# peakcrosser7/spmv-samples

Measured on AMD Instinct MI355X. Metric: GFLOP/s (2*nnz/t) and achieved HBM GB/s, CSR SpMV fp32, 1/2/4/8 MI355X, higher is better.
Workload: dtype f32

## Files before the change

include/mi355_spmv.h:

```cpp
#ifndef MI355_SPMV_H
#define MI355_SPMV_H

#include <stddef.h>
#include <stdint.h>

#ifdef __cplusplus
extern "C" {
#endif

#define MI355_SPMV_VERSION 310
#define MI355_SPMV_HAS_PATTERN 1
#define MI355_SPMV_HAS_MULTI 1
#define MI355_SPMV_HAS_MULTI_SEMIRING 1
#define MI355_SPMV_HAS_MULTI_HALF 1
#define MI355_SPMV_HAS_HALF_MATRIX 1

enum {
    MI355_SPMV_OK = 0,
    MI355_SPMV_EINVAL = 1,
    MI355_SPMV_ENOTSUP = 2,
    MI355_SPMV_EHIP = 3,
    MI355_SPMV_ENOMEM = 4,
    MI355_SPMV_ENODEV = 5
};
// ... 82 lines not shown
    int64_t grid_blocks;
    int64_t tile_items;
    int64_t n_tiles;
    int64_t rows_per_chunk;
    int64_t scratch_bytes;
    int32_t n_kernels;
    int32_t window_elems;
    int32_t window_segments;
    char main_kernel[64];
    int32_t balanced_chunks;
    int32_t rows_cap;
    int64_t n_chunks;
    char knobs[160];
    int64_t packed_index_bytes;
    int64_t packed_index_escapes;
} mi355_spmv_plan_info;
int mi355_spmv_plan_get_info(const mi355_spmv_plan* plan, mi355_spmv_plan_info* info);

typedef struct mi355_spmv_plan_shape {
    int32_t struct_bytes;
    int32_t kind, off_type, val_type;
    int32_t n_rows, n_cols;
    int64_t nnz;
    int32_t lanes_per_row, elems_per_lane, block_threads;
    int32_t balanced_chunks, rows_cap, giant_rows_enabled;
    int64_t rows_per_chunk, n_chunks, bal_k, bal_q, giant_len;
    int32_t window_elems, window_bytes, window_from_band, window_segments, probe_ok, long_steps;
    int64_t band_lo, band_hi, seg_lo[4], seg_hi[4];
    int32_t window_sweep;
    int32_t small_plain;
// ... 162 lines not shown
```

spmv-samples_amd/capi.py:

```python
import ctypes as C
import os

import torch

_HERE = os.path.dirname(os.path.abspath(__file__))
LIB_PATH = os.environ.get("MI355_SPMV_LIB") or os.path.join(_HERE, "lib", "libmi355spmv.so")

KINDS = {"vector": 0, "merge": 1, "light": 2, "auto": 100}
KIND_NAMES = {0: "vector", 1: "merge", 2: "light"}
LABELS = {"hip_vector": "vector", "hip_merge": "merge", "hip_light": "light", "hip_auto": "auto"}
OFF_TYPES = {torch.int32: (0, "i32"), torch.int64: (1, "i64")}
VAL_TYPES = {torch.float32: (0, "f32"), torch.float64: (1, "f64"), torch.int32: (2, "i32")}
VAL_PATTERN = 3
MAT_TYPES = {torch.float16: (4, "f16"), torch.bfloat16: (5, "bf16")}
PLAN_REUSE_STRUCTURE = 1
PLAN_NO_INDEX_COPY = 2
SEMIRINGS = {"plus_times": 0, "min_plus": 1, "max_times": 2, "max_plus": 3, "or_and": 4}

EXPORTS = (
    ["mi355_spmv_%s_%s_%s" % (k, o, v) for k in KINDS for o in ("i32", "i64") for v in ("f32", "f64")]
    + ["mi355_spmv_merge_genl_%s_%s" % (o, v) for o in ("i32", "i64") for v in ("f32", "f64", "i32")]
    + ["mi355_spmv_plan_set_semiring", "mi355_spmv_plan_set_alpha_beta"]
    + ["mi355_spmv_plan_create", "mi355_spmv_plan_execute", "mi355_spmv_plan_destroy",
       "mi355_spmv_plan_get_info", "mi355_spmv_stream_synchronize", "mi355_spmv_plan_merge_coords", "mi355_spmv_version",
# ... 14 lines not shown
    + ["mi355_spmv_multi_%s_%s" % (o, v) for o in ("i32", "i64") for v in ("f32", "f64")]
    + ["mi355_spmv_multi_" + n for n in ("create_typed", "set_semiring", "get_types")]
    + ["mi355_spmv_multi_%s_%s_%s" % (g, o, v) for g in ("genl", "pattern") for o in ("i32", "i64") for v in ("f32", "f64", "i32")]
    + ["mi355_spmv_multi_create_half"]
    + ["mi355_spmv_multi_half_%s_%s" % (o, v) for o in ("i32", "i64") for v in ("f16", "bf16")]
)


class PlanInfo(C.Structure):
    _fields_ = [("kind", C.c_int32), ("off_type", C.c_int32), ("val_type", C.c_int32),
                ("lanes_per_row", C.c_int32), ("elems_per_lane", C.c_int32), ("block_threads", C.c_int32),
                ("grid_blocks", C.c_int64), ("tile_items", C.c_int64), ("n_tiles", C.c_int64),
                ("rows_per_chunk", C.c_int64), ("scratch_bytes", C.c_int64), ("n_kernels", C.c_int32),
                ("window_elems", C.c_int32), ("window_segments", C.c_int32), ("main_kernel", C.c_char * 64),
                ("balanced_chunks", C.c_int32), ("rows_cap", C.c_int32), ("n_chunks", C.c_int64),
                ("knobs", C.c_char * 160), ("packed_index_bytes", C.c_int64), ("packed_index_escapes", C.c_int64)]

    def as_dict(self):
        d = {n: getattr(self, n) for n, _ in self._fields_}
        d["main_kernel"] = d["main_kernel"].decode()
        d["knobs"] = d["knobs"].decode()
        return d


class PlanShape(C.Structure):
    _fields_ = [("struct_bytes", C.c_int32), ("kind", C.c_int32), ("off_type", C.c_int32), ("val_type", C.c_int32),
                ("n_rows", C.c_int32), ("n_cols", C.c_int32), ("nnz", C.c_int64),
                ("lanes_per_row", C.c_int32), ("elems_per_lane", C.c_int32), ("block_threads", C.c_int32),
                ("balanced_chunks", C.c_int32), ("rows_cap", C.c_int32), ("giant_rows_enabled", C.c_int32),
                ("rows_per_chunk", C.c_int64), ("n_chunks", C.c_int64), ("bal_k", C.c_int64), ("bal_q", C.c_int64),
                ("giant_len", C.c_int64),
# ... 803 lines not shown
```

spmv-samples_amd/csrc/capi.hip:

```cpp

#include <algorithm>
#include <cstdarg>
#include <mutex>
#include <new>
#include <type_traits>

#include "common.hpp"

struct mi355_spmv_plan {
    mi355::Plan p;
    int acquired_on = -1;
    int asked_kind = -1;
};

namespace mi355 {

static thread_local char g_err[512] = "";

void set_error(const char* fmt, ...) {
    va_list ap;
    va_start(ap, fmt);
    vsnprintf(g_err, sizeof(g_err), fmt, ap);
    va_end(ap);
}
// ... 495 lines not shown
    if (!h || !info) { set_error("plan_get_info: null argument"); return MI355_SPMV_EINVAL; }
    const Plan& p = h->p;
    memset(info, 0, sizeof(*info));
    info->kind = p.kind; info->off_type = p.off_type; info->val_type = p.val_type;
    info->lanes_per_row = p.lanes_per_row;
    info->elems_per_lane = p.elems_per_lane;
    info->block_threads = (p.kind == MI355_KIND_MERGE && p.merge_rows && p.mat_type != MI355_VAL_PATTERN)
                              ? p.mr_block : (p.block_threads > 0 ? p.block_threads : kBlock);
    info->grid_blocks = p.grid_blocks;
    info->tile_items = p.tile_items;
    info->n_tiles = p.n_tiles;
    info->rows_per_chunk = p.rows_per_chunk;
    info->scratch_bytes = (int64_t)(p.scratch_bytes + p.packed_bytes);
    info->packed_index_bytes = (int64_t)p.packed_bytes;
    info->packed_index_escapes = p.packed_escapes;
    info->n_kernels = p.n_kernels;
    const bool windowed = p.window_elems > 0 && !(is_half_matrix(p.mat_type) && !half_matrix_chunked(p));
    info->window_elems = windowed ? p.window_elems : 0;
    info->window_segments = windowed ? (p.n_seg >= 2 ? p.n_seg : 1) : 0;
    snprintf(info->main_kernel, sizeof(info->main_kernel), "%s", p.main_kernel);
    info->balanced_chunks = p.balanced ? 1 : 0;
    info->rows_cap = p.rows_cap;
    info->n_chunks = p.n_chunks;
    snprintf(info->knobs, sizeof(info->knobs), "%s", p.knob.text);
    return MI355_SPMV_OK;
}

int mi355_spmv_plan_get_mat_type(const mi355_spmv_plan* h, int* mat_type) {
    if (!h || !mat_type) { set_error("plan_get_mat_type: null argument"); return MI355_SPMV_EINVAL; }
    *mat_type = h->p.mat_type;
// ... 105 lines not shown
```

spmv-samples_amd/csrc/common.hpp:

```cpp
#pragma once

#include <hip/hip_runtime.h>

#include <cstdint>
#include <cstdio>
#include <cstring>
#include <mutex>

#include "../../include/mi355_spmv.h"

namespace mi355 {

constexpr int kWave = 64;
constexpr int kBlock = 256;
constexpr int kMaxGiantRows = 1024;
constexpr int64_t kGiantRow = 65536;
constexpr int64_t kGiantSlice = 32768;
inline int64_t giant_slice_for(int64_t giant_len) {
    int64_t s = (giant_len / 2) & ~int64_t(1023);
    if (s < 2048) s = 2048;
    return s < kGiantSlice ? s : kGiantSlice;
}
constexpr int kWideBlock = 512;
constexpr int kHugeBlock = 1024;
// ... 116 lines not shown
    int n_giant = 0;
    int64_t giant_len = 0;
    int64_t n_giant_slices = 0;
    int32_t* giant_row = nullptr;
    int64_t* giant_slice_first = nullptr;
    void* giant_partial = nullptr;
    void* scratch = nullptr;
    size_t scratch_bytes = 0;
    size_t scratch_capacity = 0;
    int32_t* tile_row = nullptr;
    int64_t* tile_nnz = nullptr;
    int32_t* carry_row = nullptr;
    void* carry_val = nullptr;
    unsigned long long* counters = nullptr;
    uint16_t* packed_index = nullptr;
    size_t packed_bytes = 0;
    int64_t packed_escapes = 0;
    bool light_dequeue_once = false;
    int n_kernels = 0;
    bool small_plain = false;
    char main_kernel[64] = "";
};
static_assert(sizeof(Plan) <= 2048, "Plan (1 096 bytes) holds what executes and reports read; plan-time buffers are locals of plan_create");

constexpr int kProbePerRow = 32;
struct ProbeSamples {
    int n = 0;
    bool sorted = false;
    int64_t off[kBlock * kProbePerRow];
};
struct GiantRowList {
    int32_t row[kMaxGiantRows];
    int64_t slice_first[kMaxGiantRows + 1];
};
struct BlockSpec {
    const mi355_spmv_plan_shape* whole;
    int64_t row_begin, chunk_begin, n_chunks, nnz_begin_whole;
    int phase;
// ... 57 lines not shown
```

spmv-samples_amd/csrc/csr_vector.hip:

```cpp

#include <cstdlib>

#include "common.hpp"
#include "row_dot.hpp"
#include "row_launch.hpp"
#include "xwindow.hpp"

namespace mi355 {

template <int BLOCK, int T, int R, int NSEG, bool ADAPT, typename val_t, bool PACKED = false>
__global__ __launch_bounds__(BLOCK, (BLOCK >= kWideBlock || R == 2 ? 4 : 3)) void csr_vector_window_kernel(
    int32_t n_rows, int32_t n_cols, int64_t nnz, const ApView Ap, const int32_t* __restrict__ Aj,
    const val_t* __restrict__ Ax, const val_t* __restrict__ x, val_t* __restrict__ y, ChunkMap cmap,
    int32_t window_cap, BandHint hint, SegmentPlan segs, const uint16_t* __restrict__ Aj16, val_t alpha, val_t beta) {
    static_assert(!PACKED || (NSEG == 1 && !ADAPT), "the packed index exists for one band-placed window and equal-row chunks");
    extern __shared__ __attribute__((aligned(16))) unsigned char s_dyn[];
    __shared__ int s_red[2];
    ChunkScratch<val_t> scr(s_dyn, window_cap, cmap.rows_cap);
    scr.alpha = alpha;
    scr.beta = beta;
    scr.long_steps = cmap.long_steps;
    scr.giant_len = cmap.giant_len;
    const unsigned chunk = cmap.table ? blockIdx.x : xcd_contiguous_id(blockIdx.x, gridDim.x);
    int64_t rb, re;
    cmap.range(chunk, n_rows, rb, re);
    if (rb >= re) return;
    bool fits;
    const int64_t base = stage_chunk_bounds<val_t>(scr, rb, re, Ap, cmap.rel_limit, fits);
    if (!fits) {
// ... 7 lines not shown
    const int32_t nnz_c = int32_t(left < kRel32Limit + 32768 ? left : kRel32Limit + 32768);
    if constexpr (NSEG > 1) {
        auto stage = [&] { return stage_x_segments<val_t>(rb, re, n_cols, x, scr.s_x, window_cap, segs); };
        chunk_rows_any<BLOCK, T, R, true, ADAPT, val_t>(rb, re, nnz_c, Aj_c, Ax_c, x, y, stage, scr);
    } else {
        auto first_last = [&](int64_t r, int& first, int& last) {
            const int32_t s = scr.s_b[r - rb], e = scr.s_b[r - rb + 1];
            if (e <= s) return false;
            first = Aj_c[s];
            last = Aj_c[e - 1];
            return true;
        };
        auto stage = [&] {
            return stage_x_window<val_t>(rb, re, n_cols, first_last, x, scr.s_x, window_cap, s_red, hint);
        };
        if constexpr (PACKED)
            chunk_rows_any<BLOCK, T, R, true, false, val_t, decltype(stage)&, false, true>(rb, re, nnz_c, Aj_c, Ax_c, x, y, stage,
                                                                                          scr, Aj16 + base);
        else
            chunk_rows_any<BLOCK, T, R, NSEG == 1, ADAPT, val_t>(rb, re, nnz_c, Aj_c, Ax_c, x, y, stage, scr);
    }
}

template <int T, int R, typename val_t>
__global__ __launch_bounds__(kHugeBlock, 4) void csr_vector_sweep_kernel(
    int32_t n_rows, int32_t n_cols, int64_t nnz, const ApView Ap, const int32_t* __restrict__ Aj,
    const val_t* __restrict__ Ax, const val_t* __restrict__ x, val_t* __restrict__ y, ChunkMap cmap,
    int32_t window_cap, BandHint hint, val_t alpha, val_t beta) {
    extern __shared__ __attribute__((aligned(16))) unsigned char s_dyn[];
    ChunkScratch<val_t> scr(s_dyn, window_cap, cmap.rows_cap);
    scr.alpha = alpha;
    scr.beta = beta;
// ... 25 lines not shown
    off_t start = 0, end = 0;
    if (live) {
        start = Ap[row];
        end = Ap[row + 1];
    }
    val_t sum = row_partial<T, off_t, val_t>(start, end, lane, Aj, Ax, x);
    sum = vector_reduce<T, val_t>(sum);
    if (live && lane == 0) y[row] = (beta != val_t(0)) ? alpha * sum + beta * y[row] : alpha * sum;
}

struct VectorRows {
    static constexpr const char* name = "csr_vector";
    static constexpr bool kCounters = false;
    static constexpr bool kPlainKnob = true;
    static constexpr bool kPackedIndex = true;
    template <int BLOCK, int T, int R, int NSEG, bool ADAPT, typename val_t, bool PACKED = false>
    static auto window() { return csr_vector_window_kernel<BLOCK, T, R, NSEG, ADAPT, val_t, PACKED>; }
    template <int T, int R, typename val_t>
    static auto sweep() { return csr_vector_sweep_kernel<T, R, val_t>; }
    template <typename off_t, typename val_t>
    static int plain(const Plan& p, const off_t* Ap, const val_t* Ax, const val_t* x, val_t* y, hipStream_t s) {
        return launch_vector_plain<off_t, val_t>(p, Ap, Ax, x, y, s);
    }
};

template <typename off_t, typename val_t>
int launch_vector_plain(const Plan& p, const off_t* Ap, const val_t* Ax, const val_t* x, val_t* y, hipStream_t s) {
    return with_lanes(p, VectorRows::name, [&](auto lanes) -> int {
        constexpr int T = decltype(lanes)::value, rows_per_block = kBlock / T;
        const dim3 grid((unsigned)((int64_t(p.n_rows) + rows_per_block - 1) / rows_per_block)), block(kBlock);
        hipLaunchKernelGGL((csr_vector_kernel<T, off_t, val_t>), grid, block, 0, s, p.n_rows, (off_t)p.nnz, Ap, p.Aj, Ax, x, y,
                           (val_t)p.alpha, (val_t)p.beta);
// ... 20 lines not shown
```

spmv-samples_amd/csrc/csr_vector_h16.hip:

```cpp

#include "common.hpp"
#include "row_dot.hpp"
#include "row_launch.hpp"
#include "xwindow.hpp"

namespace mi355 {
namespace h16 {

template <int BLOCK, int T, int R, int NSEG, bool PACKED, typename mat_t>
__global__ __launch_bounds__(BLOCK, (BLOCK >= kWideBlock || R == 2 ? 4 : 3)) void csr_vector_window_kernel(
    int32_t n_rows, int32_t n_cols, int64_t nnz, const ApView Ap, const int32_t* __restrict__ Aj,
    const mat_t* __restrict__ Ax, const float* __restrict__ x, float* __restrict__ y, ChunkMap cmap,
    int32_t window_cap, BandHint hint, const uint16_t* __restrict__ Aj16, float alpha, float beta) {
    static_assert(NSEG == 0 || NSEG == 1, "one window of x or none");
    static_assert(!PACKED || NSEG == 1, "the packed index exists for one band-placed window");
    extern __shared__ __attribute__((aligned(16))) unsigned char s_dyn[];
    __shared__ int s_red[2];
    ChunkScratch<float> scr(s_dyn, window_cap, cmap.rows_cap);
    scr.alpha = alpha;
    scr.beta = beta;
    scr.long_steps = cmap.long_steps;
    scr.giant_len = cmap.giant_len;
    const unsigned chunk = xcd_contiguous_id(blockIdx.x, gridDim.x);
    int64_t rb, re;
    cmap.range(chunk, n_rows, rb, re);
    if (rb >= re) return;
    bool fits;
    const int64_t base = stage_chunk_bounds<float>(scr, rb, re, Ap, cmap.rel_limit, fits);
    if (!fits) {
// ... 1 lines not shown
        return;
    }
    __syncthreads();
    const int32_t* const Aj_c = Aj + base;
    const mat_t* const Ax_c = Ax + base;
    const int64_t left = nnz - base;
    const int32_t nnz_c = int32_t(left < kRel32Limit + 32768 ? left : kRel32Limit + 32768);
    auto first_last = [&](int64_t r, int& first, int& last) {
        const int32_t s = scr.s_b[r - rb], e = scr.s_b[r - rb + 1];
        if (e <= s) return false;
        first = Aj_c[s];
        last = Aj_c[e - 1];
        return true;
    };
    auto stage = [&] { return stage_x_window<float>(rb, re, n_cols, first_last, x, scr.s_x, window_cap, s_red, hint); };
    chunk_rows_any<BLOCK, T, R, NSEG == 1, false, float, decltype(stage)&, false, PACKED>(rb, re, nnz_c, Aj_c, Ax_c, x, y, stage, scr,
                                                                                          PACKED ? Aj16 + base : nullptr);
}

template <int T, typename off_t, typename mat_t>
__global__ __launch_bounds__(kBlock) void csr_vector_kernel(
    int32_t n_rows, off_t nnz, const off_t* __restrict__ Ap, const int32_t* __restrict__ Aj,
    const mat_t* __restrict__ Ax, const float* __restrict__ x, float* __restrict__ y, float alpha, float beta) {
    constexpr int ROWS_PER_BLOCK = kBlock / T;
    const unsigned blk = xcd_contiguous_id(blockIdx.x, gridDim.x);
    const int lane = threadIdx.x & (T - 1);
    const int64_t row = int64_t(blk) * ROWS_PER_BLOCK + (threadIdx.x / T);
    const bool live = row < n_rows;
    off_t start = 0, end = 0;
    if (live) {
        start = Ap[row];
        end = Ap[row + 1];
// ... 33 lines not shown
        return MI355_SPMV_OK;
    });
}

template <int BLOCK, typename mat_t>
static int launch_window(const RowOperands<float, mat_t>& o) {
    const Plan& p = o.p;
    if constexpr (BLOCK >= kWideBlock) {
        if (p.window_elems <= 0) return launch_window<kBlock, mat_t>(o);
    }
    const BandHint hint{p.band_lo, p.band_hi, p.window_from_band};
    const ChunkMap cmap = chunk_map_of(p);
    auto go = [&](auto kernel) { return launch_chunked<Rows, float>(kernel, BLOCK, o, cmap, hint, (const uint16_t*)p.packed_index); };
    return with_lanes(p, Rows::name, [&](auto lanes) -> int {
        constexpr int T = decltype(lanes)::value, R = rows_in_flight(sizeof(float), T);
        if (p.packed_index && p.window_elems > 0 && p.window_from_band) return go(csr_vector_window_kernel<BLOCK, T, R, 1, true, mat_t>);
        if (p.window_elems > 0) return go(csr_vector_window_kernel<BLOCK, T, R, 1, false, mat_t>);
        if constexpr (BLOCK == kBlock) return go(csr_vector_window_kernel<BLOCK, T, R, 0, false, mat_t>);
        return MI355_SPMV_OK;
    });
}

}

template <typename off_t, typename mat_t>
int launch_vector_half(const Plan& p, const off_t* Ap, const mat_t* Ax, const float* x, float* y, hipStream_t s) {
    static_assert(sizeof(mat_t) == 2, "a 16-bit stored type");
    if (p.n_rows == 0) return MI355_SPMV_OK;
    const bool aligned = ((reinterpret_cast<uintptr_t>(p.Aj) | reinterpret_cast<uintptr_t>(x)) & 15u) == 0 &&
                         (reinterpret_cast<uintptr_t>(Ax) & 7u) == 0;
    if (!half_matrix_chunked(p) || !aligned || p.nnz < 4 || (p.knob.plain != 0 && !p.is_block))
        return h16::launch_plain<off_t, mat_t>(p, Ap, Ax, x, y, s);
    const RowOperands<float, mat_t> o{p, ApView{Ap, sizeof(off_t) == 8 ? 1 : 0}, Ax, x, y, s,
// ... 24 lines not shown
```

spmv-samples_amd/csrc/row_dot.hpp:

```cpp
#pragma once

#include <type_traits>

#include "common.hpp"

namespace mi355 {

typedef int int4v __attribute__((ext_vector_type(4)));
typedef unsigned uint2v __attribute__((ext_vector_type(2)));
constexpr unsigned kPackedEscape = 0xFFFFu;
typedef float float4v __attribute__((ext_vector_type(4)));
typedef double double4v __attribute__((ext_vector_type(4)));

template <typename val_t> struct Vec4;
template <> struct Vec4<float> { using type = float4v; };
template <> struct Vec4<double> { using type = double4v; };
template <> struct Vec4<int32_t> { using type = int4v; };
template <> struct Vec4<PatternOnes> { using type = PatternOnes; };

typedef _Float16 half4v __attribute__((ext_vector_type(4)));
template <> struct Vec4<_Float16> { using type = uint2v; };
template <> struct Vec4<Bf16> { using type = uint2v; };

template <typename val_t, typename mat_t>
// ... 45 lines not shown
```

spmv-samples_amd/csrc/row_launch.hpp:

```cpp

#pragma once

#include <type_traits>

#include "common.hpp"
#include "giant_rows.hpp"
#include "xwindow.hpp"

namespace mi355 {

template <typename F>
static int with_lanes(const Plan& p, const char* kind, F&& f) {
    switch (p.lanes_per_row) {
        case 2: return f(std::integral_constant<int, 2>());
        case 4: return f(std::integral_constant<int, 4>());
        case 8: return f(std::integral_constant<int, 8>());
        case 16: return f(std::integral_constant<int, 16>());
        case 32: return f(std::integral_constant<int, 32>());
        case 64: return f(std::integral_constant<int, 64>());
    }
    set_error("%s: bad lanes_per_row %d", kind, p.lanes_per_row);
    return MI355_SPMV_EINVAL;
}

// ... 45 lines not shown
        constexpr int R = rows_in_flight(sizeof(val_t), 2);
        const int st = p.window_elems > 0 ? go(Kind::template window<kBlock, 2, R, 1, true, val_t>())
                                          : go(Kind::template window<kBlock, 2, R, 0, true, val_t>());
        if (st != MI355_SPMV_OK) return st;
        return launch_giant_rows<off_t, val_t>(p, Ap, o.Ax, o.x, o.y, o.s);
    }
    return with_lanes(p, Kind::name, [&](auto lanes) -> int {
        constexpr int T = decltype(lanes)::value, R = rows_in_flight(sizeof(val_t), T);
        if (p.window_elems > 0 && p.n_seg >= 2) {
            if constexpr (BLOCK == kBlock) return go(Kind::template window<BLOCK, T, R, kMaxSegments, false, val_t>());
            set_error("%s: no 512-thread kernel for a multi-band window", Kind::name);
            return MI355_SPMV_EINVAL;
        }
        if constexpr (Kind::kPackedIndex) {
            if (p.packed_index && p.window_elems > 0 && p.window_from_band)
                return go(Kind::template window<BLOCK, T, R, 1, false, val_t, true>());
        }
        if (p.window_elems > 0) return go(Kind::template window<BLOCK, T, R, 1, false, val_t>());
        if constexpr (BLOCK == kBlock) return go(Kind::template window<BLOCK, T, R, 0, false, val_t>());
        return MI355_SPMV_OK;
    });
}

template <typename Kind, typename val_t>
static int launch_rows_sweep(const RowOperands<val_t>& o) {
    const Plan& p = o.p;
    const BandHint hint{p.band_lo, p.band_hi, true};
    const ChunkMap cmap{nullptr, (int32_t)p.rows_per_chunk, (int32_t)p.rows_cap, p.n_chunks, 0, int64_t(0),
                        p.knob.rel32_limit > 0 ? p.knob.rel32_limit : kRel32Limit, p.light_dequeue_once ? 1 : 0};
    const int64_t vectors = kHugeBlock / p.lanes_per_row;
    const int held = int(p.rows_per_chunk / vectors);
// ... 33 lines not shown
```

spmv-samples_amd/csrc/rows_plan.hip:

```cpp

#include <algorithm>
#include <utility>

#include "common.hpp"
#include "row_dot.hpp"
#include "xwindow.hpp"

namespace mi355 {

static int workgroups_per_cu_by_registers(const Plan& p) {
    if (p.block_threads == kHugeBlock) return 1;
    if (p.block_threads == kWideBlock) return 2;
    if (p.balanced) return p.val_type == MI355_VAL_F64 ? 4 : 3;
    return (p.val_type == MI355_VAL_F64 || p.lanes_per_row >= 16) ? 4 : 3;
}

int long_steps_for(const Plan& p) {
    if (p.knob.long_steps > 0) return p.knob.long_steps;
    return p.balanced ? 4 : kLongSteps;
}

static int pick_lanes_per_row(int64_t nnz, int64_t n_rows, int elems) {
    const int64_t mean = n_rows > 0 ? (nnz + n_rows - 1) / n_rows : 0;
    int t = 2;
// ... 226 lines not shown
    const int tid = threadIdx.x;
    if (tid < s4 - s) out[s + tid] = uint16_t(encode(Aj[s + tid]));
    if (tid < e - e4) out[e4 + tid] = uint16_t(encode(Aj[e4 + tid]));
    for (int64_t k = s4 + int64_t(tid) * 4; k < e4; k += int64_t(kBlock) * 4) {
        const int4v c = stream_load(reinterpret_cast<const int4v*>(Aj + k));
        uint2v v;
        v[0] = encode(c[0]) | (encode(c[1]) << 16);
        v[1] = encode(c[2]) | (encode(c[3]) << 16);
        *reinterpret_cast<uint2v*>(out + k) = v;
    }
#pragma unroll
    for (int o = 32; o >= 1; o >>= 1) escaped += __shfl_xor(escaped, o, kWave);
    if ((tid & (kWave - 1)) == 0 && escaped) atomicAdd(escapes, (unsigned long long)escaped);
}

int build_packed_index(Plan& p) {
    p.packed_index = nullptr;
    p.packed_bytes = 0;
    p.packed_escapes = 0;
    if (p.kind != MI355_KIND_VECTOR || (p.flags & MI355_PLAN_NO_INDEX_COPY) || p.knob.pack == 0) return MI355_SPMV_OK;
    if (p.small_plain || p.sweep || p.balanced || (p.knob.plain != 0 && !p.is_block)) return MI355_SPMV_OK;
    if (p.window_elems <= 0 || p.window_elems > 65535 || p.n_seg >= 2 || !p.window_from_band) return MI355_SPMV_OK;
    if (p.n_rows <= 0 || p.nnz < 4 || p.nnz <= p.nnz_begin || p.n_chunks < 1 || p.n_chunks > int64_t(UINT32_MAX)) return MI355_SPMV_OK;
    if ((reinterpret_cast<uintptr_t>(p.Aj) & 15u) != 0) return MI355_SPMV_OK;
    const size_t bytes = (((size_t(p.nnz_read) + 3) & ~size_t(3)) + 4) * sizeof(uint16_t);
    void* ptr = nullptr;
    if (hipMalloc(&ptr, bytes) != hipSuccess) {
        (void)hipGetLastError();
        return MI355_SPMV_OK;
    }
    const AnalysisBuffer buf;
    unsigned long long* d_escapes = reinterpret_cast<unsigned long long*>(buf.words);
    hipError_t e = d_escapes ? hipSuccess : hipErrorOutOfMemory;
    if (e == hipSuccess) e = hipMemsetAsync(ptr, 0xFF, bytes, nullptr);
    if (e == hipSuccess) e = hipMemsetAsync(d_escapes, 0, sizeof(unsigned long long), nullptr);
    if (e == hipSuccess) {
        const ApView Ap{p.Ap, p.off_type == MI355_OFF_I64 ? 1 : 0};
        const BandHint hint{p.band_lo, p.band_hi, true};
        const dim3 grid((unsigned)p.n_chunks), block(kBlock);
        if (p.val_type == MI355_VAL_F64)
            hipLaunchKernelGGL((pack_index_kernel<double>), grid, block, 0, nullptr, p.n_rows, p.n_cols, Ap, p.Aj,
                               static_cast<uint16_t*>(ptr), chunk_map_of(p), (int32_t)p.window_elems, hint, d_escapes);
        else
            hipLaunchKernelGGL((pack_index_kernel<float>), grid, block, 0, nullptr, p.n_rows, p.n_cols, Ap, p.Aj,
                               static_cast<uint16_t*>(ptr), chunk_map_of(p), (int32_t)p.window_elems, hint, d_escapes);
        e = hipGetLastError();
    }
    unsigned long long escaped = 0;
    if (e == hipSuccess) e = hipMemcpy(&escaped, d_escapes, sizeof(escaped), hipMemcpyDeviceToHost);
    if (e != hipSuccess) {
        (void)hipFree(ptr);
        set_error("build_packed_index: %s", hipGetErrorString(e));
        return MI355_SPMV_EHIP;
    }
    p.packed_index = static_cast<uint16_t*>(ptr);
    p.packed_bytes = bytes;
    p.packed_escapes = int64_t(escaped);
    return MI355_SPMV_OK;
}

static int window_budget(const Plan& p, int block_threads, int64_t rows) {
    if (block_threads == kBlock) return kWindowBytes;
    const size_t val_bytes = p.val_type == MI355_VAL_F64 ? 8 : 4;
    const int64_t avail = 63 * 1024 - int64_t(chunk_lds_bytes(0, int(rows), val_bytes));
    return int(avail < 0 ? 0 : avail);
}

static int rows_in_flight_of(const Plan& p) { return rows_in_flight(p.val_type == MI355_VAL_F64 ? 8 : 4, p.lanes_per_row); }
static bool one_band_window(const Plan& p) { return p.window_elems > 0 && p.n_seg < 2 && p.window_from_band; }

static void shrink_to_whole_rounds(Plan& p, int64_t pass) {
    if (p.knob.rows_per_chunk > 0 || p.n_seg >= 2) return;
// ... 271 lines not shown
```

spmv-samples_amd/csrc/xwindow.hpp:

```cpp
#pragma once

#include <climits>
#include <type_traits>

#include "common.hpp"
#include "row_dot.hpp"

namespace mi355 {

constexpr int kSamples = 32;

template <typename val_t>
struct XWindow {
    const val_t* s_x;
    int32_t lo;
    int32_t len;
    __device__ __forceinline__ bool find(int32_t col, unsigned& idx) const {
        const unsigned rel = unsigned(col - lo);
        const bool in = rel < unsigned(len);
        idx = in ? rel : 0u;
        return in;
    }
};

// ... 319 lines not shown
        for (int g = tid; g < full; g += BLOCK)
            __builtin_nontemporal_store(*reinterpret_cast<const v16*>(scr.s_y + g * PER16),
                                        reinterpret_cast<v16*>(yc + g * PER16));
        for (int i = full * PER16 + tid; i < n_store; i += BLOCK) yc[i] = scr.s_y[i];
    } else if (!scaled) {
        for (int i = tid; i < n_store; i += BLOCK) yc[i] = scr.s_y[i];
    } else {
        for (int i = tid; i < n_store; i += BLOCK) {
            val_t v = alpha * scr.s_y[i];
            if (beta != val_t(0)) v += beta * yc[i];
            yc[i] = v;
        }
    }
}

template <int BLOCK, int T, int R, bool WINDOW, typename val_t, bool PACKED = false, typename StageFn, typename mat_t = val_t>
__device__ __forceinline__ void chunk_rows(int64_t chunk_begin, int64_t chunk_end, int32_t nnz,
                                           const int32_t* __restrict__ Aj,
                                           const mat_t* __restrict__ Ax, const val_t* __restrict__ x,
                                           val_t* __restrict__ y, StageFn&& stage,
                                           const ChunkScratch<val_t>& scr,
                                           const uint16_t* __restrict__ Aj16 = nullptr) {
    static_assert(!PACKED || WINDOW, "a packed index is window-relative");
    using v4 = typename Vec4<val_t>::type;
    using m4 = typename Vec4<mat_t>::type;
    using col4 = typename std::conditional<PACKED, uint2v, int4v>::type;
    using off_t = int32_t;
    constexpr int VECS = BLOCK / T;
    constexpr int WAVES = BLOCK / kWave;
    constexpr int STRIDE = VECS * R;
    const off_t LONG = off_t(T) * 4 * scr.long_steps;
    const int lane = threadIdx.x & (T - 1);
    const int rows = int(chunk_end - chunk_begin);
    const int n_groups = (rows + STRIDE - 1) / STRIDE;
    const off_t nnz_vec = nnz & ~off_t(3);
    const off_t j_max = nnz_vec - 4;

    constexpr int VW = kWave / T;
    const int row_in_wave = (threadIdx.x & (kWave - 1)) / T;
    const int wave_rows0 = (threadIdx.x / kWave) * (VW * R);
#ifdef MI355_ROW_MAP_ADJACENT
    auto row_of = [&](int g, int r) { return g * STRIDE + int(threadIdx.x / T) * R + r; };
#else
    auto row_of = [&](int g, int r) { return g * STRIDE + wave_rows0 + r * VW + row_in_wave; };
#endif
    struct Group {
        col4 c[R];
        m4 a[R];
    };
    auto load_cols = [&](off_t jl) {
        if constexpr (PACKED) return stream_load(reinterpret_cast<const uint2v*>(Aj16 + jl));
        else return stream_load(reinterpret_cast<const int4v*>(Aj + jl));
    };
    struct Bounds { off_t lo[R], hi[R]; };
    auto read_bounds = [&](int g, Bounds& B) {
#pragma unroll
        for (int r = 0; r < R; ++r) {
            const int row = row_of(g, r);
            B.lo[r] = scr.s_b[min(row, rows)];
            B.hi[r] = scr.s_b[min(row + 1, rows)];
        }
    };
    auto step0 = [&](off_t lo) { return (lo & ~off_t(3)) + off_t(lane) * 4; };
    auto issue = [&](int g, Group& G) {
        Bounds B;
        read_bounds(g, B);
#pragma unroll
        for (int r = 0; r < R; ++r) {
            const off_t j0 = step0(B.lo[r]);
            off_t jl = j0 < B.hi[r] ? j0 : (B.lo[r] & ~off_t(3));
            jl = jl < j_max ? jl : j_max;
            G.c[r] = load_cols(jl);
            G.a[r] = stream_load(reinterpret_cast<const m4*>(Ax + jl));
        }
        __builtin_amdgcn_sched_barrier(0);
    };
    constexpr int DEPTH = 2;
    Group G[DEPTH];
#pragma unroll
    for (int d = 0; d < DEPTH - 1; ++d) issue(d, G[d]);
    const auto win = stage();

    auto pin4 = [](val_t (&v)[4]) { asm volatile("" : "+v"(v[0]), "+v"(v[1]), "+v"(v[2]), "+v"(v[3])); };
    auto gather4 = [&](const auto& c, val_t (&xv)[4], bool (&in)[4]) {
        constexpr bool packed_group = std::is_same<std::decay_t<decltype(c)>, uint2v>::value;
        if constexpr (PACKED) {
            unsigned idx[4];
// ... 64 lines not shown
        bool deferred[R];
        bool more = false;
#pragma unroll
        for (int r = 0; r < R; ++r) {
            const off_t len_r = B.hi[r] - B.lo[r];
            deferred[r] = len_r > LONG || (scr.giant_len > 0 && int64_t(len_r) > scr.giant_len);
            hi[r] = deferred[r] ? B.lo[r] : (B.hi[r] < nnz_vec ? B.hi[r] : nnz_vec);
            sum[r] = val_t(0);
        }
        constexpr int XB = R >= 2 ? 2 : 1;
#pragma unroll
        for (int r0 = 0; r0 < R; r0 += XB) {
            val_t xv[XB][4];
            bool in[XB][4];
#pragma unroll
            for (int b = 0; b < XB; ++b) gather4(G.c[r0 + b], xv[b], in[b]);
#pragma unroll
            for (int b = 0; b < XB; ++b) pin4(xv[b]);
#pragma unroll
            for (int b = 0; b < XB; ++b) {
                const int r = r0 + b;
                const off_t j0 = step0(B.lo[r]);
                fold4(sum[r], G.c[r], widen4<val_t, mat_t>(G.a[r]), xv[b], in[b], j0, B.lo[r], hi[r]);
                jn[r] = j0 + off_t(T) * 4;
                more |= jn[r] < hi[r];
            }
        }
        while (more) {
            col4 c2[R];
            m4 a2[R];
#pragma unroll
            for (int r = 0; r < R; ++r) {
                off_t jl = jn[r] < hi[r] ? jn[r] : (B.lo[r] & ~off_t(3));
                jl = jl < j_max ? jl : j_max;
                c2[r] = load_cols(jl);
                a2[r] = stream_load(reinterpret_cast<const m4*>(Ax + jl));
            }
            more = false;
// ... 133 lines not shown
                    val_t total = s_part[0];
#pragma unroll
                    for (int i = 1; i < WAVES; ++i) total += s_part[i];
                    scr.s_y[local] = total;
                }
                __syncthreads();
            }
        }
    }

    __syncthreads();
    store_chunk_results<BLOCK, val_t>(scr, y, chunk_begin, rows, tid2);
}

template <int BLOCK, int T, int R, bool WINDOW, bool ADAPT, typename val_t, typename StageFn, bool REGULAR = false,
          bool PACKED = false, typename mat_t = val_t>
__device__ __forceinline__ void chunk_rows_any(int64_t chunk_begin, int64_t chunk_end, int32_t nnz,
                                               const int32_t* __restrict__ Aj,
                                               const mat_t* __restrict__ Ax, const val_t* __restrict__ x,
                                               val_t* __restrict__ y, StageFn&& stage,
                                               const ChunkScratch<val_t>& scr,
                                               const uint16_t* __restrict__ Aj16 = nullptr) {
    static_assert(!PACKED || !ADAPT, "packed plans have equal-row chunks of one vector width");
    if constexpr (!ADAPT) {
        chunk_rows<BLOCK, T, R, WINDOW, val_t, PACKED>(chunk_begin, chunk_end, nnz, Aj, Ax, x, y, stage, scr, Aj16);
    } else {
        const int rows = int(chunk_end - chunk_begin);
        const int32_t mean = (scr.s_b[rows] - scr.s_b[0]) / int32_t(rows > 0 ? rows : 1);
        if constexpr (REGULAR) {
            if (mean <= 8) chunk_rows<BLOCK, 2, R, WINDOW, val_t>(chunk_begin, chunk_end, nnz, Aj, Ax, x, y, stage, scr);
            else if (mean <= 16) chunk_rows<BLOCK, 4, R, WINDOW, val_t>(chunk_begin, chunk_end, nnz, Aj, Ax, x, y, stage, scr);
            else if (mean <= 32) chunk_rows<BLOCK, 8, R, WINDOW, val_t>(chunk_begin, chunk_end, nnz, Aj, Ax, x, y, stage, scr);
            else if (mean <= 64) chunk_rows<BLOCK, 16, R, WINDOW, val_t>(chunk_begin, chunk_end, nnz, Aj, Ax, x, y, stage, scr);
            else chunk_rows<BLOCK, 32, R, WINDOW, val_t>(chunk_begin, chunk_end, nnz, Aj, Ax, x, y, stage, scr);
            return;
        }
        if (mean <= 16) chunk_rows<BLOCK, 2, R, WINDOW, val_t>(chunk_begin, chunk_end, nnz, Aj, Ax, x, y, stage, scr);
        else if (mean <= 64) chunk_rows<BLOCK, 8, R, WINDOW, val_t>(chunk_begin, chunk_end, nnz, Aj, Ax, x, y, stage, scr);
        else chunk_rows<BLOCK, 32, R, WINDOW, val_t>(chunk_begin, chunk_end, nnz, Aj, Ax, x, y, stage, scr);
    }
// ... 158 lines not shown
```

Before: 1913.

## Add row-pair interleaved packed column index layout for windowed vector kernel

```diff
diff --git a/include/mi355_spmv.h b/include/mi355_spmv.h
--- a/include/mi355_spmv.h
+++ b/include/mi355_spmv.h
@@ -120,6 +120,8 @@
     char knobs[160];
     int64_t packed_index_bytes;
     int64_t packed_index_escapes;
+    int32_t packed_index_layout;
+    int64_t packed_index_late;
 } mi355_spmv_plan_info;
 int mi355_spmv_plan_get_info(const mi355_spmv_plan* plan, mi355_spmv_plan_info* info);
 
diff --git a/spmv-samples_amd/capi.py b/spmv-samples_amd/capi.py
--- a/spmv-samples_amd/capi.py
+++ b/spmv-samples_amd/capi.py
@@ -52,7 +52,8 @@
                 ("rows_per_chunk", C.c_int64), ("scratch_bytes", C.c_int64), ("n_kernels", C.c_int32),
                 ("window_elems", C.c_int32), ("window_segments", C.c_int32), ("main_kernel", C.c_char * 64),
                 ("balanced_chunks", C.c_int32), ("rows_cap", C.c_int32), ("n_chunks", C.c_int64),
-                ("knobs", C.c_char * 160), ("packed_index_bytes", C.c_int64), ("packed_index_escapes", C.c_int64)]
+                ("knobs", C.c_char * 160), ("packed_index_bytes", C.c_int64), ("packed_index_escapes", C.c_int64),
+                ("packed_index_layout", C.c_int32), ("packed_index_late", C.c_int64)]
 
     def as_dict(self):
         d = {n: getattr(self, n) for n, _ in self._fields_}
diff --git a/spmv-samples_amd/csrc/capi.hip b/spmv-samples_amd/csrc/capi.hip
--- a/spmv-samples_amd/csrc/capi.hip
+++ b/spmv-samples_amd/csrc/capi.hip
@@ -533,6 +533,8 @@
     info->scratch_bytes = (int64_t)(p.scratch_bytes + p.packed_bytes);
     info->packed_index_bytes = (int64_t)p.packed_bytes;
     info->packed_index_escapes = p.packed_escapes;
+    info->packed_index_layout = p.packed_index ? p.packed_form : 0;
+    info->packed_index_late = p.packed_late;
     info->n_kernels = p.n_kernels;
     const bool windowed = p.window_elems > 0 && !(is_half_matrix(p.mat_type) && !half_matrix_chunked(p));
     info->window_elems = windowed ? p.window_elems : 0;
diff --git a/spmv-samples_amd/csrc/common.hpp b/spmv-samples_amd/csrc/common.hpp
--- a/spmv-samples_amd/csrc/common.hpp
+++ b/spmv-samples_amd/csrc/common.hpp
@@ -8,6 +8,7 @@
 #include <mutex>
 
 #include "../../include/mi355_spmv.h"
+#include "pair_layout.hpp"
 
 namespace mi355 {
 
@@ -154,6 +155,8 @@
     void* carry_val = nullptr;
     unsigned long long* counters = nullptr;
     uint16_t* packed_index = nullptr;
+    int packed_form = 0;
+    int64_t packed_late = 0;
     size_t packed_bytes = 0;
     int64_t packed_escapes = 0;
     bool light_dequeue_once = false;
@@ -161,7 +164,7 @@
     bool small_plain = false;
     char main_kernel[64] = "";
 };
-static_assert(sizeof(Plan) <= 2048, "Plan (1 096 bytes) holds what executes and reports read; plan-time buffers are locals of plan_create");
+static_assert(sizeof(Plan) <= 2048, "Plan (1 112 bytes) holds what executes and reports read; plan-time buffers are locals of plan_create");
 
 constexpr int kProbePerRow = 32;
 struct ProbeSamples {
diff --git a/spmv-samples_amd/csrc/csr_vector.hip b/spmv-samples_amd/csrc/csr_vector.hip
--- a/spmv-samples_amd/csrc/csr_vector.hip
+++ b/spmv-samples_amd/csrc/csr_vector.hip
@@ -8,11 +8,12 @@
 
 namespace mi355 {
 
-template <int BLOCK, int T, int R, int NSEG, bool ADAPT, typename val_t, bool PACKED = false>
+template <int BLOCK, int T, int R, int NSEG, bool ADAPT, typename val_t, PackedForm FORM = kPackedNone>
 __global__ __launch_bounds__(BLOCK, (BLOCK >= kWideBlock || R == 2 ? 4 : 3)) void csr_vector_window_kernel(
     int32_t n_rows, int32_t n_cols, int64_t nnz, const ApView Ap, const int32_t* __restrict__ Aj,
     const val_t* __restrict__ Ax, const val_t* __restrict__ x, val_t* __restrict__ y, ChunkMap cmap,
     int32_t window_cap, BandHint hint, SegmentPlan segs, const uint16_t* __restrict__ Aj16, val_t alpha, val_t beta) {
+    constexpr bool PACKED = FORM != kPackedNone;
     static_assert(!PACKED || (NSEG == 1 && !ADAPT), "the packed index exists for one band-placed window and equal-row chunks");
     extern __shared__ __attribute__((aligned(16))) unsigned char s_dyn[];
     __shared__ int s_red[2];
@@ -50,8 +51,13 @@
         auto stage = [&] {
             return stage_x_window<val_t>(rb, re, n_cols, first_last, x, scr.s_x, window_cap, s_red, hint);
         };
-        if constexpr (PACKED)
-            chunk_rows_any<BLOCK, T, R, true, false, val_t, decltype(stage)&, false, true>(rb, re, nnz_c, Aj_c, Ax_c, x, y, stage,
+        if constexpr (FORM == kPackedPairs) {
+            const int64_t first = pair_unit_of_row(rb, T);
+            chunk_rows_any<BLOCK, T, R, true, false, val_t, decltype(stage)&, false, FORM>(
+                rb, re, nnz_c, Aj_c, Ax_c, x, y, stage, scr, Aj16 + first * kPairUnitSlots,
+                pair_last_unit_in_chunk(pair_units(n_rows, T), first));
+        } else if constexpr (PACKED)
+            chunk_rows_any<BLOCK, T, R, true, false, val_t, decltype(stage)&, false, FORM>(rb, re, nnz_c, Aj_c, Ax_c, x, y, stage,
                                                                                           scr, Aj16 + base);
         else
             chunk_rows_any<BLOCK, T, R, NSEG == 1, ADAPT, val_t>(rb, re, nnz_c, Aj_c, Ax_c, x, y, stage, scr);
@@ -107,8 +113,8 @@
     static constexpr bool kCounters = false;
     static constexpr bool kPlainKnob = true;
     static constexpr bool kPackedIndex = true;
-    template <int BLOCK, int T, int R, int NSEG, bool ADAPT, typename val_t, bool PACKED = false>
-    static auto window() { return csr_vector_window_kernel<BLOCK, T, R, NSEG, ADAPT, val_t, PACKED>; }
+    template <int BLOCK, int T, int R, int NSEG, bool ADAPT, typename val_t, PackedForm FORM = kPackedNone>
+    static auto window() { return csr_vector_window_kernel<BLOCK, T, R, NSEG, ADAPT, val_t, FORM>; }
     template <int T, int R, typename val_t>
     static auto sweep() { return csr_vector_sweep_kernel<T, R, val_t>; }
     template <typename off_t, typename val_t>
diff --git a/spmv-samples_amd/csrc/csr_vector_h16.hip b/spmv-samples_amd/csrc/csr_vector_h16.hip
--- a/spmv-samples_amd/csrc/csr_vector_h16.hip
+++ b/spmv-samples_amd/csrc/csr_vector_h16.hip
@@ -7,12 +7,13 @@
 namespace mi355 {
 namespace h16 {
 
-template <int BLOCK, int T, int R, int NSEG, bool PACKED, typename mat_t>
+template <int BLOCK, int T, int R, int NSEG, PackedForm FORM, typename mat_t>
 __global__ __launch_bounds__(BLOCK, (BLOCK >= kWideBlock || R == 2 ? 4 : 3)) void csr_vector_window_kernel(
     int32_t n_rows, int32_t n_cols, int64_t nnz, const ApView Ap, const int32_t* __restrict__ Aj,
     const mat_t* __restrict__ Ax, const float* __restrict__ x, float* __restrict__ y, ChunkMap cmap,
     int32_t window_cap, BandHint hint, const uint16_t* __restrict__ Aj16, float alpha, float beta) {
     static_assert(NSEG == 0 || NSEG == 1, "one window of x or none");
+    constexpr bool PACKED = FORM != kPackedNone;
     static_assert(!PACKED || NSEG == 1, "the packed index exists for one band-placed window");
     extern __shared__ __attribute__((aligned(16))) unsigned char s_dyn[];
     __shared__ int s_red[2];
@@ -44,8 +45,14 @@
         return true;
     };
     auto stage = [&] { return stage_x_window<float>(rb, re, n_cols, first_last, x, scr.s_x, window_cap, s_red, hint); };
-    chunk_rows_any<BLOCK, T, R, NSEG == 1, false, float, decltype(stage)&, false, PACKED>(rb, re, nnz_c, Aj_c, Ax_c, x, y, stage, scr,
-                                                                                          PACKED ? Aj16 + base : nullptr);
+    if constexpr (FORM == kPackedPairs) {
+        const int64_t first = pair_unit_of_row(rb, T);
+        chunk_rows_any<BLOCK, T, R, true, false, float, decltype(stage)&, false, FORM>(
+            rb, re, nnz_c, Aj_c, Ax_c, x, y, stage, scr, Aj16 + first * kPairUnitSlots,
+            pair_last_unit_in_chunk(pair_units(n_rows, T), first));
+    } else
+        chunk_rows_any<BLOCK, T, R, NSEG == 1, false, float, decltype(stage)&, false, FORM>(rb, re, nnz_c, Aj_c, Ax_c, x, y, stage, scr,
+                                                                                            PACKED ? Aj16 + base : nullptr);
 }
 
 template <int T, typename off_t, typename mat_t>
@@ -109,9 +116,11 @@
     auto go = [&](auto kernel) { return launch_chunked<Rows, float>(kernel, BLOCK, o, cmap, hint, (const uint16_t*)p.packed_index); };
     return with_lanes(p, Rows::name, [&](auto lanes) -> int {
         constexpr int T = decltype(lanes)::value, R = rows_in_flight(sizeof(float), T);
-        if (p.packed_index && p.window_elems > 0 && p.window_from_band) return go(csr_vector_window_kernel<BLOCK, T, R, 1, true, mat_t>);
-        if (p.window_elems > 0) return go(csr_vector_window_kernel<BLOCK, T, R, 1, false, mat_t>);
-        if constexpr (BLOCK == kBlock) return go(csr_vector_window_kernel<BLOCK, T, R, 0, false, mat_t>);
+        if (p.packed_index && p.window_elems > 0 && p.window_from_band)
+            return p.packed_form == kPackedPairs ? go(csr_vector_window_kernel<BLOCK, T, R, 1, kPackedPairs, mat_t>)
+                                                 : go(csr_vector_window_kernel<BLOCK, T, R, 1, kPackedNatural, mat_t>);
+        if (p.window_elems > 0) return go(csr_vector_window_kernel<BLOCK, T, R, 1, kPackedNone, mat_t>);
+        if constexpr (BLOCK == kBlock) return go(csr_vector_window_kernel<BLOCK, T, R, 0, kPackedNone, mat_t>);
         return MI355_SPMV_OK;
     });
 }
diff --git a/spmv-samples_amd/csrc/pair_layout.hpp b/spmv-samples_amd/csrc/pair_layout.hpp
--- /dev/null
+++ b/spmv-samples_amd/csrc/pair_layout.hpp
@@ -0,0 +1,50 @@
+#pragma once
+
+#include <cstdint>
+
+#if defined(__HIPCC__)
+#define MI355_PAIR_FN __host__ __device__ constexpr
+#else
+#define MI355_PAIR_FN constexpr
+#endif
+
+namespace mi355 {
+
+enum PackedForm : int { kPackedNone = 0, kPackedNatural = 1, kPackedPairs = 2 };
+
+constexpr int kPairWave = 64;
+constexpr int kPairUnitSlots = 8;
+
+MI355_PAIR_FN int64_t pair_block_rows(int T) { return 2 * int64_t(kPairWave / T); }
+
+MI355_PAIR_FN int64_t pair_slot(int64_t rho, int T, int l, int e) {
+    const int64_t vw = kPairWave / T;
+    return ((rho / (2 * vw)) * kPairWave + (rho % vw) * T + l) * kPairUnitSlots + ((rho / vw) & 1) * 4 + e;
+}
+
+MI355_PAIR_FN int64_t pair_units(int64_t n_rows, int T) {
+    const int64_t vw = kPairWave / T;
+    const int64_t rem = n_rows % (2 * vw);
+    return (n_rows / (2 * vw)) * kPairWave + (rem < vw ? rem : vw) * T;
+}
+
+MI355_PAIR_FN int64_t pair_unit_of_row(int64_t rho, int T) { return (rho / pair_block_rows(T)) * kPairWave; }
+
+MI355_PAIR_FN int32_t pair_unit_in_chunk(int g, int wave, int lane64, int p, int T, int R, int rows_per_group) {
+    const int vw = kPairWave / T;
+    return (g * (rows_per_group / (2 * vw)) + wave * (R / 2) + p) * kPairWave + lane64;
+}
+
+MI355_PAIR_FN int32_t pair_last_unit_in_chunk(int64_t total_units, int64_t chunk_first_unit) {
+    const int64_t last = total_units - 1 - chunk_first_unit;
+    return int32_t(last < INT32_MAX ? last : INT32_MAX);
+}
+MI355_PAIR_FN int32_t pair_clamp_unit(int32_t unit, int32_t last_unit) { return unit < last_unit ? unit : last_unit; }
+
+MI355_PAIR_FN bool pair_rule(int64_t n_rows, int T, int64_t nnz, int64_t late) {
+    const int64_t br = pair_block_rows(T);
+    const int64_t rows16 = (n_rows + br - 1) / br * br;
+    return 16 * (8 * int64_t(T) * rows16 + 4 * late) <= 2 * nnz * 17;
+}
+
+}
diff --git a/spmv-samples_amd/csrc/row_dot.hpp b/spmv-samples_amd/csrc/row_dot.hpp
--- a/spmv-samples_amd/csrc/row_dot.hpp
+++ b/spmv-samples_amd/csrc/row_dot.hpp
@@ -8,6 +8,7 @@
 
 typedef int int4v __attribute__((ext_vector_type(4)));
 typedef unsigned uint2v __attribute__((ext_vector_type(2)));
+typedef unsigned uint4v __attribute__((ext_vector_type(4)));
 constexpr unsigned kPackedEscape = 0xFFFFu;
 typedef float float4v __attribute__((ext_vector_type(4)));
 typedef double double4v __attribute__((ext_vector_type(4)));
diff --git a/spmv-samples_amd/csrc/row_launch.hpp b/spmv-samples_amd/csrc/row_launch.hpp
--- a/spmv-samples_amd/csrc/row_launch.hpp
+++ b/spmv-samples_amd/csrc/row_launch.hpp
@@ -83,7 +83,8 @@
         }
         if constexpr (Kind::kPackedIndex) {
             if (p.packed_index && p.window_elems > 0 && p.window_from_band)
-                return go(Kind::template window<BLOCK, T, R, 1, false, val_t, true>());
+                return p.packed_form == kPackedPairs ? go(Kind::template window<BLOCK, T, R, 1, false, val_t, kPackedPairs>())
+                                                     : go(Kind::template window<BLOCK, T, R, 1, false, val_t, kPackedNatural>());
         }
         if (p.window_elems > 0) return go(Kind::template window<BLOCK, T, R, 1, false, val_t>());
         if constexpr (BLOCK == kBlock) return go(Kind::template window<BLOCK, T, R, 0, false, val_t>());
diff --git a/spmv-samples_amd/csrc/rows_plan.hip b/spmv-samples_amd/csrc/rows_plan.hip
--- a/spmv-samples_amd/csrc/rows_plan.hip
+++ b/spmv-samples_amd/csrc/rows_plan.hip
@@ -264,16 +264,107 @@
     if ((tid & (kWave - 1)) == 0 && escaped) atomicAdd(escapes, (unsigned long long)escaped);
 }
 
+template <typename val_t>
+__global__ __launch_bounds__(kBlock) void pack_pairs_kernel(int32_t n_rows, int32_t n_cols, const ApView Ap,
+                                                            const int32_t* __restrict__ Aj, uint16_t* __restrict__ out,
+                                                            ChunkMap cmap, int32_t window_cap, BandHint hint, int T,
+                                                            unsigned long long* escapes) {
+    int64_t rb, re;
+    cmap.range(blockIdx.x, n_rows, rb, re);
+    if (rb >= re) return;
+    const WindowSpan w = band_window<val_t>(rb, re, n_cols, window_cap, hint);
+    unsigned escaped = 0;
+    auto encode = [&](int32_t col) -> unsigned {
+        const unsigned rel = unsigned(col - w.lo);
+        const bool in = rel < unsigned(w.len);
+        escaped += in ? 0u : 1u;
+        return in ? rel : kPackedEscape;
+    };
+    const int vw = kWave / T;
+    const int64_t first = pair_unit_of_row(rb, T);
+    const int64_t here = (re - rb + 2 * vw - 1) / (2 * vw) * kWave, left = pair_units(n_rows, T) - first;
+    const int n_units = int(here < left ? here : left);
+    const int tid = threadIdx.x;
+    for (int u = tid; u < n_units; u += kBlock) {
+        const int l64 = u & (kWave - 1), v = l64 / T, l = l64 % T;
+        unsigned idx[8];
+#pragma unroll
+        for (int h = 0; h < 2; ++h) {
+            const int64_t rho = rb + int64_t(u / kWave) * 2 * vw + h * vw + v;
+#pragma unroll
+            for (int e = 0; e < 4; ++e) idx[4 * h + e] = kPackedEscape;
+            if (rho >= re) continue;
+            const int64_t lo = Ap.at(rho), hi = Ap.at(rho + 1);
+            int64_t k0 = (lo & ~int64_t(3)) + 4 * l;
+#pragma unroll
+            for (int e = 0; e < 4; ++e)
+                if (k0 + e >= lo && k0 + e < hi) idx[4 * h + e] = encode(Aj[k0 + e]);
+            for (k0 += 4 * T; k0 < hi; k0 += 4 * T)
+                for (int e = 0; e < 4 && k0 + e < hi; ++e) (void)encode(Aj[k0 + e]);
+        }
+        uint4v unit;
+#pragma unroll
+        for (int i = 0; i < 4; ++i) unit[i] = idx[2 * i] | (idx[2 * i + 1] << 16);
+        *reinterpret_cast<uint4v*>(out + (first + u) * kPairUnitSlots) = unit;
+    }
+#pragma unroll
+    for (int o = 32; o >= 1; o >>= 1) escaped += __shfl_xor(escaped, o, kWave);
+    if ((tid & (kWave - 1)) == 0 && escaped) atomicAdd(escapes, (unsigned long long)escaped);
+}
+
+__global__ __launch_bounds__(kBlock) void late_count_kernel(int32_t n_rows, const ApView Ap, int T, unsigned long long* out) {
+    unsigned long long late = 0;
+    for (int64_t r = int64_t(blockIdx.x) * kBlock + threadIdx.x; r < n_rows; r += int64_t(gridDim.x) * kBlock) {
+        const int64_t lo = Ap.at(r), over = Ap.at(r + 1) - ((lo & ~int64_t(3)) + 4 * T);
+        late += over > 0 ? (unsigned long long)over : 0ull;
+    }
+#pragma unroll
+    for (int o = 32; o >= 1; o >>= 1) late += __shfl_xor(late, o, kWave);
+    if ((threadIdx.x & (kWave - 1)) == 0 && late) atomicAdd(out, late);
+}
+
+static int wants_row_pairs(Plan& p, const ApView& Ap, bool& pairs) {
+    pairs = false;
+    p.packed_late = 0;
+    const int T = p.lanes_per_row;
+    if (p.knob.pack != 3 || T < 2 || T > kWave || rows_in_flight(p.val_type == MI355_VAL_F64 ? 8 : 4, T) % 2 != 0) return MI355_SPMV_OK;
+    if (p.n_chunks > 1 && p.rows_per_chunk % pair_block_rows(T) != 0) return MI355_SPMV_OK;
+    const AnalysisBuffer buf;
+    unsigned long long* d_late = reinterpret_cast<unsigned long long*>(buf.words);
+    if (!d_late) { set_error("build_packed_index: no device scratch"); return MI355_SPMV_ENOMEM; }
+    hipError_t e = hipMemsetAsync(d_late, 0, sizeof(unsigned long long), nullptr);
+    if (e == hipSuccess) {
+        const unsigned g = unsigned(std::min<int64_t>((int64_t(p.n_rows) + kBlock - 1) / kBlock, 2048));
+        hipLaunchKernelGGL(late_count_kernel, dim3(g), dim3(kBlock), 0, nullptr, p.n_rows, Ap, T, d_late);
+        e = hipGetLastError();
+    }
+    unsigned long long late = 0;
+    if (e == hipSuccess) e = hipMemcpy(&late, d_late, sizeof(late), hipMemcpyDeviceToHost);
+    if (e != hipSuccess) {
+        set_error("build_packed_index: %s", hipGetErrorString(e));
+        return MI355_SPMV_EHIP;
+    }
+    p.packed_late = int64_t(late);
+    pairs = pair_rule(p.n_rows, T, p.nnz - p.nnz_begin, p.packed_late);
+    return MI355_SPMV_OK;
+}
+
 int build_packed_index(Plan& p) {
     p.packed_index = nullptr;
     p.packed_bytes = 0;
     p.packed_escapes = 0;
+    p.packed_form = kPackedNone;
+    p.packed_late = 0;
     if (p.kind != MI355_KIND_VECTOR || (p.flags & MI355_PLAN_NO_INDEX_COPY) || p.knob.pack == 0) return MI355_SPMV_OK;
     if (p.small_plain || p.sweep || p.balanced || (p.knob.plain != 0 && !p.is_block)) return MI355_SPMV_OK;
     if (p.window_elems <= 0 || p.window_elems > 65535 || p.n_seg >= 2 || !p.window_from_band) return MI355_SPMV_OK;
     if (p.n_rows <= 0 || p.nnz < 4 || p.nnz <= p.nnz_begin || p.n_chunks < 1 || p.n_chunks > int64_t(UINT32_MAX)) return MI355_SPMV_OK;
     if ((reinterpret_cast<uintptr_t>(p.Aj) & 15u) != 0) return MI355_SPMV_OK;
-    const size_t bytes = (((size_t(p.nnz_read) + 3) & ~size_t(3)) + 4) * sizeof(uint16_t);
+    const ApView Ap{p.Ap, p.off_type == MI355_OFF_I64 ? 1 : 0};
+    bool pairs = false;
+    if (const int st = wants_row_pairs(p, Ap, pairs)) return st;
+    const size_t bytes = pairs ? size_t(pair_units(p.n_rows, p.lanes_per_row)) * 16
+                               : (((size_t(p.nnz_read) + 3) & ~size_t(3)) + 4) * sizeof(uint16_t);
     void* ptr = nullptr;
     if (hipMalloc(&ptr, bytes) != hipSuccess) {
         (void)hipGetLastError();
@@ -282,13 +373,18 @@
     const AnalysisBuffer buf;
     unsigned long long* d_escapes = reinterpret_cast<unsigned long long*>(buf.words);
     hipError_t e = d_escapes ? hipSuccess : hipErrorOutOfMemory;
-    if (e == hipSuccess) e = hipMemsetAsync(ptr, 0xFF, bytes, nullptr);
+    if (e == hipSuccess && !pairs) e = hipMemsetAsync(ptr, 0xFF, bytes, nullptr);
     if (e == hipSuccess) e = hipMemsetAsync(d_escapes, 0, sizeof(unsigned long long), nullptr);
     if (e == hipSuccess) {
-        const ApView Ap{p.Ap, p.off_type == MI355_OFF_I64 ? 1 : 0};
         const BandHint hint{p.band_lo, p.band_hi, true};
         const dim3 grid((unsigned)p.n_chunks), block(kBlock);
-        if (p.val_type == MI355_VAL_F64)
+        if (pairs && p.val_type == MI355_VAL_F64)
+            hipLaunchKernelGGL((pack_pairs_kernel<double>), grid, block, 0, nullptr, p.n_rows, p.n_cols, Ap, p.Aj,
+                               static_cast<uint16_t*>(ptr), chunk_map_of(p), (int32_t)p.window_elems, hint, p.lanes_per_row, d_escapes);
+        else if (pairs)
+            hipLaunchKernelGGL((pack_pairs_kernel<float>), grid, block, 0, nullptr, p.n_rows, p.n_cols, Ap, p.Aj,
+                               static_cast<uint16_t*>(ptr), chunk_map_of(p), (int32_t)p.window_elems, hint, p.lanes_per_row, d_escapes);
+        else if (p.val_type == MI355_VAL_F64)
             hipLaunchKernelGGL((pack_index_kernel<double>), grid, block, 0, nullptr, p.n_rows, p.n_cols, Ap, p.Aj,
                                static_cast<uint16_t*>(ptr), chunk_map_of(p), (int32_t)p.window_elems, hint, d_escapes);
         else
@@ -306,6 +402,7 @@
     p.packed_index = static_cast<uint16_t*>(ptr);
     p.packed_bytes = bytes;
     p.packed_escapes = int64_t(escaped);
+    p.packed_form = pairs ? kPackedPairs : kPackedNatural;
     return MI355_SPMV_OK;
 }
 
diff --git a/spmv-samples_amd/csrc/xwindow.hpp b/spmv-samples_amd/csrc/xwindow.hpp
--- a/spmv-samples_amd/csrc/xwindow.hpp
+++ b/spmv-samples_amd/csrc/xwindow.hpp
@@ -4,6 +4,7 @@
 #include <type_traits>
 
 #include "common.hpp"
+#include "pair_layout.hpp"
 #include "row_dot.hpp"
 
 namespace mi355 {
@@ -357,17 +358,22 @@
     }
 }
 
-template <int BLOCK, int T, int R, bool WINDOW, typename val_t, bool PACKED = false, typename StageFn, typename mat_t = val_t>
+template <int BLOCK, int T, int R, bool WINDOW, typename val_t, PackedForm FORM = kPackedNone, typename StageFn, typename mat_t = val_t>
 __device__ __forceinline__ void chunk_rows(int64_t chunk_begin, int64_t chunk_end, int32_t nnz,
                                            const int32_t* __restrict__ Aj,
                                            const mat_t* __restrict__ Ax, const val_t* __restrict__ x,
                                            val_t* __restrict__ y, StageFn&& stage,
                                            const ChunkScratch<val_t>& scr,
-                                           const uint16_t* __restrict__ Aj16 = nullptr) {
+                                           const uint16_t* __restrict__ Aj16 = nullptr, int32_t idx_last = 0) {
+    constexpr bool PACKED = FORM != kPackedNone;
+    constexpr bool PAIRS = FORM == kPackedPairs;
     static_assert(!PACKED || WINDOW, "a packed index is window-relative");
+    static_assert(!PAIRS || R % 2 == 0, "row pairs: slots 2p and 2p + 1 share a 16-byte unit");
     using v4 = typename Vec4<val_t>::type;
     using m4 = typename Vec4<mat_t>::type;
-    using col4 = typename std::conditional<PACKED, uint2v, int4v>::type;
+    using col4 = typename std::conditional<PACKED && !PAIRS, uint2v, int4v>::type;
+    using idx0 = typename std::conditional<PAIRS, uint4v, col4>::type;
+    constexpr int NIDX = PAIRS ? R / 2 : R;
     using off_t = int32_t;
     constexpr int VECS = BLOCK / T;
     constexpr int WAVES = BLOCK / kWave;
@@ -388,12 +394,16 @@
     auto row_of = [&](int g, int r) { return g * STRIDE + wave_rows0 + r * VW + row_in_wave; };
 #endif
     struct Group {
-        col4 c[R];
+        idx0 c[NIDX];
         m4 a[R];
     };
     auto load_cols = [&](off_t jl) {
-        if constexpr (PACKED) return stream_load(reinterpret_cast<const uint2v*>(Aj16 + jl));
+        if constexpr (PACKED && !PAIRS) return stream_load(reinterpret_cast<const uint2v*>(Aj16 + jl));
         else return stream_load(reinterpret_cast<const int4v*>(Aj + jl));
+    };
+    auto cols0 = [](const Group& G, int r) {
+        if constexpr (PAIRS) return uint2v{G.c[r >> 1][2 * (r & 1)], G.c[r >> 1][2 * (r & 1) + 1]};
+        else return G.c[r];
     };
     struct Bounds { off_t lo[R], hi[R]; };
     auto read_bounds = [&](int g, Bounds& B) {
@@ -406,6 +416,15 @@
     };
     auto step0 = [&](off_t lo) { return (lo & ~off_t(3)) + off_t(lane) * 4; };
     auto issue = [&](int g, Group& G) {
+        if constexpr (PAIRS) {
+            int tid = threadIdx.x;
+            asm volatile("" : "+v"(tid));
+#pragma unroll
+            for (int p = 0; p < R / 2; ++p) {
+                const int32_t u = pair_clamp_unit(pair_unit_in_chunk(g, tid / kWave, tid & (kWave - 1), p, T, R, STRIDE), idx_last);
+                G.c[p] = stream_load(reinterpret_cast<const uint4v*>(Aj16) + u);
+            }
+        }
         Bounds B;
         read_bounds(g, B);
 #pragma unroll
@@ -413,7 +432,7 @@
             const off_t j0 = step0(B.lo[r]);
             off_t jl = j0 < B.hi[r] ? j0 : (B.lo[r] & ~off_t(3));
             jl = jl < j_max ? jl : j_max;
-            G.c[r] = load_cols(jl);
+            if constexpr (!PAIRS) G.c[r] = load_cols(jl);
             G.a[r] = stream_load(reinterpret_cast<const m4*>(Ax + jl));
         }
         __builtin_amdgcn_sched_barrier(0);
@@ -508,14 +527,14 @@
             val_t xv[XB][4];
             bool in[XB][4];
 #pragma unroll
-            for (int b = 0; b < XB; ++b) gather4(G.c[r0 + b], xv[b], in[b]);
+            for (int b = 0; b < XB; ++b) gather4(cols0(G, r0 + b), xv[b], in[b]);
 #pragma unroll
             for (int b = 0; b < XB; ++b) pin4(xv[b]);
 #pragma unroll
             for (int b = 0; b < XB; ++b) {
                 const int r = r0 + b;
                 const off_t j0 = step0(B.lo[r]);
-                fold4(sum[r], G.c[r], widen4<val_t, mat_t>(G.a[r]), xv[b], in[b], j0, B.lo[r], hi[r]);
+                fold4(sum[r], cols0(G, r), widen4<val_t, mat_t>(G.a[r]), xv[b], in[b], j0, B.lo[r], hi[r]);
                 jn[r] = j0 + off_t(T) * 4;
                 more |= jn[r] < hi[r];
             }
@@ -679,16 +698,16 @@
 }
 
 template <int BLOCK, int T, int R, bool WINDOW, bool ADAPT, typename val_t, typename StageFn, bool REGULAR = false,
-          bool PACKED = false, typename mat_t = val_t>
+          PackedForm FORM = kPackedNone, typename mat_t = val_t>
 __device__ __forceinline__ void chunk_rows_any(int64_t chunk_begin, int64_t chunk_end, int32_t nnz,
                                                const int32_t* __restrict__ Aj,
                                                const mat_t* __restrict__ Ax, const val_t* __restrict__ x,
                                                val_t* __restrict__ y, StageFn&& stage,
                                                const ChunkScratch<val_t>& scr,
-                                               const uint16_t* __restrict__ Aj16 = nullptr) {
-    static_assert(!PACKED || !ADAPT, "packed plans have equal-row chunks of one vector width");
+                                               const uint16_t* __restrict__ Aj16 = nullptr, int32_t idx_last = 0) {
+    static_assert(FORM == kPackedNone || !ADAPT, "packed plans have equal-row chunks of one vector width");
     if constexpr (!ADAPT) {
-        chunk_rows<BLOCK, T, R, WINDOW, val_t, PACKED>(chunk_begin, chunk_end, nnz, Aj, Ax, x, y, stage, scr, Aj16);
+        chunk_rows<BLOCK, T, R, WINDOW, val_t, FORM>(chunk_begin, chunk_end, nnz, Aj, Ax, x, y, stage, scr, Aj16, idx_last);
     } else {
         const int rows = int(chunk_end - chunk_begin);
         const int32_t mean = (scr.s_b[rows] - scr.s_b[0]) / int32_t(rows > 0 ? rows : 1);
```

Result: slower. 1867 (-2.4%).
